# xkuubix/MonteCarlo-Gated-MIL

Measured on AMD Instinct MI355X. Metric: bags/sec × MCDO-samples (T=100) at N=2048,d=512; 1/2/4/8-GPU + %HBM roofline, higher is better.
Workload: dtype bf16

## Files before the change

montecarlo-gated-mil_amd/csrc/mcgmil_fused.hip:

```cpp
#define MCGMIL_KERNELS_TEMPLATES_ONLY
#include "../../include/mcgmil.h"
#include "mcgmil_kernels.h"
#include "mcgmil_error.h"
#include "mcgmil_fused.h"


namespace mcgmil {

__global__ __launch_bounds__(1024) void plan_regions_kernel(const int32_t* bag_off, int B, int T,
                                                            int cap, int32_t* region_off) {
    __shared__ int part[1024];
    const int tid = threadIdx.x;
    const int per = (B + 1023) / 1024;
    const int b0 = tid * per, b1 = b0 + per < B ? b0 + per : B;
    int sum = 0;
    for (int b = b0; b < b1; ++b) {
        const int ts = region_t_groups(bag_off[b + 1] - bag_off[b], T, cap);
        sum += (T + ts - 1) / ts;
    }
    part[tid] = sum;
    __syncthreads();
    for (int o = 1; o < 1024; o <<= 1) {
        const int v = tid >= o ? part[tid - o] : 0;
        __syncthreads();
        part[tid] += v;
        __syncthreads();
    }
    int run = part[tid] - sum;
    for (int b = b0; b < b1; ++b) {
        region_off[b] = run;
        const int ts = region_t_groups(bag_off[b + 1] - bag_off[b], T, cap);
        run += (T + ts - 1) / ts;
    }
    if (tid == 1023) region_off[B] = part[1023];
}

}

namespace mcgmil_detail {

long long fused_regions(const mcgmil::GateParams& gp, long long total_rows, int cap, bool estimate) {
    if (gp.uniform_rows > 0) {
        const int ts = mcgmil::region_t_groups(gp.uniform_rows, gp.T, cap);
        return (long long)gp.B * ((gp.T + ts - 1) / ts);
    }
    if (estimate) return (long long)gp.T * total_rows / cap;
    return (2ll * gp.T * total_rows + cap - 1) / cap + gp.B + 1;
}

namespace {

template <typename E, int PPW, int MAXC, bool ONE>
int launch(const mcgmil::GateParams& gp, long long total_rows, hipStream_t s) {
    constexpr int cap = mcgmil::fused_cap<MAXC>();
    const bool affine = mcgmil::fused_affine(gp.uniform_rows, cap);
    auto* k = affine ? (gp.clock ? &mcgmil::gate_fused_kernel<E, PPW, MAXC, ONE, true>
                                 : &mcgmil::gate_fused_kernel<E, PPW, MAXC, ONE>)
                     : (gp.clock ? &mcgmil::gate_fused_table_kernel<E, PPW, MAXC, ONE, true>
                                 : &mcgmil::gate_fused_table_kernel<E, PPW, MAXC, ONE>);
    if (int rc = raise_lds_limit(reinterpret_cast<const void*>(k), "gate_fused_kernel LDS limit")) return rc;
    if (gp.uniform_rows <= 0) {
        hipLaunchKernelGGL(mcgmil::plan_regions_kernel, dim3(1), dim3(1024), 0, s, gp.bag_off, gp.B,
                           gp.T, cap, const_cast<int32_t*>(gp.region_off));
        hipError_t e = hipGetLastError();
        if (e != hipSuccess) return hip_fail(e, "plan_regions_kernel launch");
    }
    const long long grid = fused_regions(gp, total_rows, cap, false);
    if (grid == 0) return MCGMIL_OK;
    if (grid > 0x7fffffffll) return fail(MCGMIL_E_UNSUPPORTED, "too many regions for one launch");
    const size_t lds = mcgmil::fused_kernel_lds_bytes<E, MAXC>(gp.L);
    if (lds > 160 * 1024) return fail(MCGMIL_E_UNSUPPORTED, "fused kernel: L too large for its LDS");
    hipLaunchKernelGGL(k, dim3((unsigned)grid), dim3(mcgmil::kGateThreads), lds, s, gp);
    hipError_t e = hipGetLastError();
    return e == hipSuccess ? MCGMIL_OK : hip_fail(e, "gate_fused_kernel launch");
}

template <typename E, int MAXC>
int launch_maxc(const mcgmil::GateParams& gp, int ppw, bool one, long long total_rows, hipStream_t s) {
    if (ppw == 1) return one ? launch<E, 1, MAXC, true>(gp, total_rows, s) : launch<E, 1, MAXC, false>(gp, total_rows, s);
    return one ? launch<E, 2, MAXC, true>(gp, total_rows, s) : launch<E, 2, MAXC, false>(gp, total_rows, s);
}

}

int launch_gate_fused(const mcgmil::GateParams& gp, bool bf16, int ppw, int maxc, bool one,
                      long long total_rows, hipStream_t s) {
    if (bf16) return maxc == 2 ? launch_maxc<__bf16, 2>(gp, ppw, one, total_rows, s)
                               : launch_maxc<__bf16, 4>(gp, ppw, one, total_rows, s);
    return maxc == 2 ? launch_maxc<float, 2>(gp, ppw, one, total_rows, s)
                     : launch_maxc<float, 4>(gp, ppw, one, total_rows, s);
}

}
```

montecarlo-gated-mil_amd/csrc/mcgmil_kernels.h:

```cpp
#pragma once
#include "mcgmil_device.h"

namespace mcgmil {

struct GateParams {
    const void* H;
    long long ldh;
    const int32_t* bag_off;
    int B, T, L, D, C, G, P;
    long long total_samples;
    const void* Wp;
    uint32_t wp_bytes;
    const float* bv;
    const float* bu;
    const float* wa;
    const float* ba;
    float sf, sa;
    uint32_t thr_f, thr_a;
    uint32_t thrx_f;
    uint32_t k0, k1;
    uint32_t bag_base;
    int t_base;
    const uint32_t* bag_ids;
    const int32_t* tile_bag;
    int uniform_rows;
    const uint8_t* keep_feat;
    const uint8_t* keep_att;
    float* logits;
    float* zz;
    float* Y;
    float* A;
    const int32_t* region_off;
    int region_t;
    unsigned long long* stamps;
    unsigned long long* clock;
    long long tile_row0;
};

constexpr int kClockSlots = 1024;
__device__ __forceinline__ void clock_probe(const GateParams& p, int i) {
    if (p.clock && threadIdx.x == 0 && blockIdx.x < (unsigned)kClockSlots) {
        const unsigned long long t = __builtin_amdgcn_s_memtime();
        const unsigned long long r = __builtin_amdgcn_s_memrealtime();
        p.clock[(size_t)blockIdx.x * 4 + 2 * i] = t;
        p.clock[(size_t)blockIdx.x * 4 + 2 * i + 1] = r;
    }
}

#ifdef MCGMIL_STAMPS
#define MCGMIL_STAMP(p, i)                                                                 \
    do {                                                                                    \
        __builtin_amdgcn_sched_barrier(0);                                                  \
        if (threadIdx.x == 0 && (p).stamps)                                                 \
            (p).stamps[(size_t)blockIdx.x * 8 + (i)] = __builtin_amdgcn_s_memtime();        \
        __builtin_amdgcn_sched_barrier(0);                                                  \
    } while (0)
#else
#define MCGMIL_STAMP(p, i) do {} while (0)
#endif


constexpr int kGateThreads = 512;
constexpr int kGateWaves = kGateThreads / kWave;
constexpr int kRowInfo = 6;


template <int BM, int RV = BM>
__device__ __forceinline__ void fill_row_table(const GateParams& p, long long R0, int* rinfo) {
    const int tid = threadIdx.x;
    if (tid >= BM) return;
    const long long R = tid < RV ? R0 + tid : p.total_samples;
    int hrow = -1, t = 0, n = 0, bag = 0, Nb = 0;
    const bool narrow = p.total_samples <= 0xFFFFFFFFll;
    if (R < p.total_samples && p.uniform_rows > 0) {
        const long long per_bag = (long long)p.T * p.uniform_rows;
        Nb = p.uniform_rows;
        if (narrow) {
            const uint32_t r = (uint32_t)R, pb = (uint32_t)per_bag;
            bag = (int)(r / pb);
            const uint32_t local = r - (uint32_t)bag * pb;
            t = (int)(local / (uint32_t)Nb);
            n = (int)(local - (uint32_t)t * (uint32_t)Nb);
        } else {
// ... 11 lines not shown
            bag = find_bag(p.bag_off, p.B, p.T, R);
        }
        const int ob = p.bag_off[bag];
        Nb = p.bag_off[bag + 1] - ob;
        const long long local = R - (long long)p.T * ob;
        if (narrow) {
            t = (int)((uint32_t)local / (uint32_t)Nb);
            n = (int)((uint32_t)local - (uint32_t)t * (uint32_t)Nb);
        } else {
            t = (int)(local / Nb);
            n = (int)(local - (long long)t * Nb);
        }
        hrow = ob + n;
    }
    int* ri = rinfo + kRowInfo * tid;
    ri[0] = hrow; ri[1] = t; ri[2] = n; ri[3] = bag; ri[4] = Nb;
    ri[5] = (int)(p.bag_ids ? p.bag_ids[bag] : p.bag_base + (uint32_t)bag);
}

#ifndef MCGMIL_KERNELS_TEMPLATES_ONLY
__global__ void plan_tiles_kernel(const int32_t* bag_off, int B, int T, long long total_samples,
                                  int BM, long long tiles, int32_t* tile_bag) {
    const long long i = (long long)blockIdx.x * blockDim.x + threadIdx.x;
    if (i >= tiles) return;
    const long long R = i * BM;
    tile_bag[i] = R < total_samples ? find_bag(bag_off, B, T, R) : 0;
}
#endif

__device__ __forceinline__ float gated_product_scaled(float ax, float by) {
    ax = fminf(fmaxf(ax, -43.280851226668903f), 43.280851226668903f);
    const float a = __builtin_amdgcn_exp2f(ax);
    const float b = __builtin_amdgcn_exp2f(by);
    const float ia = 1.0f + a;
    return (1.0f - a) * __builtin_amdgcn_rcpf(fmaf(ia, b, ia));
}

#ifndef MCGMIL_DIAG
#define MCGMIL_DIAG 0
#endif
#ifndef MCGMIL_PHILOX_ROUNDS
#define MCGMIL_PHILOX_ROUNDS 10
#endif

constexpr float kM2Log2e = -2.8853900817779268f;
constexpr float kMLog2e = -1.4426950408889634f;

struct HeadVec { f32x4 bv, bu, wa; };

template <int PPW>
__device__ __forceinline__ void load_head_vectors(const GateParams& p, int q0, int lane,
                                                  HeadVec (&hv)[PPW]) {
    const int DB = p.D >> 4;
#pragma unroll
    for (int jp = 0; jp < PPW; ++jp) {
        const int q = q0 + jp < p.P ? q0 + jp : p.P - 1;
        const int g = q / DB, db = q - g * DB;
        const int d0 = db * 16 + 4 * (lane >> 4);
        hv[jp].bv = *reinterpret_cast<const f32x4*>(p.bv + (size_t)g * p.D + d0) * kM2Log2e;
        hv[jp].bu = *reinterpret_cast<const f32x4*>(p.bu + (size_t)g * p.D + d0) * kMLog2e;
        hv[jp].wa = *reinterpret_cast<const f32x4*>(p.wa + (size_t)g * p.D + d0);
    }
}

struct Region {
    int bag, t0, t1, Nb, ob;
    int ntiles;
    long long S, rows;
};

constexpr int kFusedTiles = 32;
constexpr int kFusedHv = 256;
struct alignas(16) FusedConst {
    Region rg;
    uint32_t bagctr;
    int pad0;
    float ba[4];
    int cls[8];
    int pad1[8];
    int4 tile[kFusedTiles];
    float hv[3][kFusedHv];
};

#ifndef MCGMIL_FUSED_HV_LDS
#define MCGMIL_FUSED_HV_LDS 1
#endif
template <int PPW>
__device__ __forceinline__ void load_head_vectors_lds(const FusedConst* fc, int P, int q0, int lane,
                                                      HeadVec (&hv)[PPW]) {
#pragma unroll
    for (int jp = 0; jp < PPW; ++jp) {
        const int q = q0 + jp < P ? q0 + jp : P - 1;
        const int d = 16 * q + 4 * (lane >> 4);
        hv[jp].bv = *reinterpret_cast<const f32x4*>(fc->hv[0] + d);
        hv[jp].bu = *reinterpret_cast<const f32x4*>(fc->hv[1] + d);
        hv[jp].wa = *reinterpret_cast<const f32x4*>(fc->hv[2] + d);
    }
}

template <int RT, int PPW, int MAXC, bool ONE_CLASS, int RTV = RT>
__device__ __forceinline__ void fold_pairs(const GateParams& p, const f32x4 (&acc)[RT][2 * PPW],
                                           int q0, int lane, float (&part)[MAXC][RT],
                                           const HeadVec* pre = nullptr) {
    const int DB = p.D >> 4;
    const float av_s = p.sf * kM2Log2e, au_s = p.sf * kMLog2e;
#pragma unroll
    for (int jp = 0; jp < PPW; ++jp) {
        const int q = q0 + jp;
        if (q >= p.P) break;
        const int col = 16 * q + 4 * (lane >> 4);
        const int g = ONE_CLASS ? 0 : q / DB;
        const int d0 = col - g * p.D;
        f32x4 bvv, buv;
        f32x4 coef[MAXC];
        if (ONE_CLASS && pre) {
            bvv = pre[jp].bv;
            buv = pre[jp].bu;
            coef[0] = pre[jp].wa;
#pragma unroll
            for (int c = 1; c < MAXC; ++c) coef[c] = f32x4{0.f, 0.f, 0.f, 0.f};
        } else {
            bvv = *reinterpret_cast<const f32x4*>(p.bv + col);
            buv = *reinterpret_cast<const f32x4*>(p.bu + col);
            bvv *= kM2Log2e;
            buv *= kMLog2e;
#pragma unroll
            for (int c = 0; c < MAXC; ++c) {
                const int cc = ONE_CLASS ? g : c;
                const bool use = ONE_CLASS ? (c == 0) : ((c < p.C) && (p.G == 1 || c == g));
                const f32x4 w = *reinterpret_cast<const f32x4*>(p.wa + (size_t)(use ? cc : 0) * p.D + d0);
                coef[c] = use ? w : f32x4{0.f, 0.f, 0.f, 0.f};
            }
        }
#pragma unroll
        for (int rt = 0; rt < RTV; ++rt) {
#pragma unroll
            for (int v = 0; v < 4; ++v) {
                const float ax = fmaf(acc[rt][2 * jp][v], av_s, bvv[v]);
                const float by = fmaf(acc[rt][2 * jp + 1][v], au_s, buv[v]);
                if constexpr (ONE_CLASS) {
#if MCGMIL_DIAG & 8
                    part[0][rt] = fmaf(fmaf(ax, coef[0][v], by), ax, part[0][rt]);
                    continue;
#endif
                    const float a = __builtin_amdgcn_exp2f(fminf(fmaxf(ax, -43.280851226668903f),
                                                                 43.280851226668903f));
                    const float b = __builtin_amdgcn_exp2f(by);
                    const float ia = 1.0f + a;
                    const float r = __builtin_amdgcn_rcpf(fmaf(ia, b, ia));
                    part[0][rt] = fmaf(fmaf(-a, coef[0][v], coef[0][v]), r, part[0][rt]);
                } else {
                    const float pr = gated_product_scaled(ax, by);
#pragma unroll
                    for (int c = 0; c < MAXC; ++c) part[c][rt] = fmaf(pr, coef[c][v], part[c][rt]);
                }
            }
        }
    }
}

template <int BM, int MAXC>
__host__ __device__ constexpr int red_floats() { return kGateWaves * MAXC * 4 * BM; }

template <int BM, int MAXC, int ROWS = 16, bool AFFINE = false>
__device__ __forceinline__ void finish_scores(const GateParams& p, long long R0,
                                              float (&part)[MAXC][BM / ROWS], f32x4 zacc,
                                              bool zwave, float* red, float* zred,
                                              const int* rinfo, int one_class, int waves_per_gate,
                                              bool have_keep, bool keep, float* lg_out,
                                              float* z_out, long long obase,
                                              const FusedConst* fc = nullptr, int tile = 0) {
    constexpr int RT = BM / ROWS;
    constexpr int NG = 64 / ROWS;
    const int tid = threadIdx.x, lane = tid & 63, wave = tid >> 6;
    const int ncls = one_class < 0 ? MAXC : 1;
#pragma unroll
    for (int c = 0; c < MAXC; ++c) {
        if (c >= ncls) break;
        const int cls = one_class < 0 ? c : one_class;
        if (cls >= MAXC) break;
        float* dst = red + ((size_t)(wave * MAXC + cls) * NG + lane / ROWS) * BM + (lane % ROWS);
#pragma unroll
        for (int q = 0; q < RT; ++q) dst[ROWS * q] = part[c][q];
    }
    if (zwave && lane < 16) {
#pragma unroll
        for (int c = 0; c < MAXC; ++c) zred[c * BM + wave * 16 + lane] = zacc[c];
    }
    MCGMIL_STAMP(p, 5);
    __syncthreads();
    MCGMIL_STAMP(p, 6);
    const int r = wave * 16 + (lane & 15), c = lane >> 4;
    if (r >= BM || c >= p.C) return;
    int t, n, bag, Nb;
    uint32_t bagc;
    size_t orow;
    float bias;
    if constexpr (AFFINE) {
        const int4 tl = fc->tile[tile];
        t = tl.x, n = tl.y + r, bag = fc->rg.bag, Nb = fc->rg.Nb;
        bagc = fc->bagctr;
        orow = (size_t)(tl.z + r);
        bias = fc->ba[c];
    } else {
        const int* ri = rinfo + kRowInfo * r;
        if (ri[0] < 0) return;
        t = ri[1], n = ri[2], bag = ri[3], Nb = ri[4];
        bagc = (uint32_t)ri[5];
        orow = (size_t)(R0 + r - obase);
        bias = p.ba[c];
    }
    float s = 0.f;
    const int nw = waves_per_gate ? waves_per_gate : kGateWaves;
    for (int k = 0; k < nw; ++k) {
        const int w = waves_per_gate ? c * waves_per_gate + k : k;
        const float* src = red + (size_t)(w * MAXC + c) * NG * BM + r;
#pragma unroll
        for (int g = 0; g < NG; ++g) s += src[g * BM];
    }
    s += bias;
    if (p.keep_att) {
        const size_t abase = (size_t)p.T * p.C * (size_t)p.bag_off[bag];
        keep = p.keep_att[abase + ((size_t)t * p.C + c) * Nb + n] != 0;
    } else if (!have_keep) {
        keep = attention_keep(p.k0, p.k1, bagc, (uint32_t)(p.t_base + t), (uint32_t)c,
                              (uint32_t)n, p.thr_a);
    }
    const size_t o = orow * p.C + c;
    lg_out[o] = s * (keep ? p.sa : 0.f);
    z_out[o] = zred[c * BM + r] * p.sf;
}

constexpr int kSoftmaxRows = 16;

#ifndef MCGMIL_NT_A
#define MCGMIL_NT_A 1
#endif
__device__ __forceinline__ void store_a(float* dst, float v) {
#if MCGMIL_NT_A
    __builtin_nontemporal_store(v, dst);
#else
    *dst = v;
#endif
}

__device__ __forceinline__ void softmax_group(int ltid, bool active, int Nb, int C, const float* lg,
                                              const float* zz, float* Ao, float* Yo, float* sred) {
    const int tid = ltid, lane = ltid & 63, wave = ltid >> 6;
    if (Nb == 0) {
        if (active && tid < C) Yo[tid] = 0.f;
        return;
    }
    const int Nl = active ? Nb : 0;
    if (C == 2 && Nb <= 256 * kSoftmaxRows) {
        float (*sred2)[4] = reinterpret_cast<float (*)[4]>(sred);
        float e0[kSoftmaxRows], e1[kSoftmaxRows];
        float2 zr[kSoftmaxRows];
        float m0 = -INFINITY, m1 = -INFINITY;
#pragma unroll
        for (int k = 0; k < kSoftmaxRows; ++k) {
            const int n = tid + 256 * k;
            float2 l = make_float2(-INFINITY, -INFINITY);
            zr[k] = make_float2(0.f, 0.f);
            if (n < Nl) {
                l = *reinterpret_cast<const float2*>(lg + (size_t)n * 2);
                zr[k] = *reinterpret_cast<const float2*>(zz + (size_t)n * 2);
            }
            e0[k] = l.x;
            e1[k] = l.y;
            m0 = fmaxf(m0, e0[k]);
            m1 = fmaxf(m1, e1[k]);
        }
        m0 = wave_max(m0);
        m1 = wave_max(m1);
        if (lane == 0) { sred2[0][wave] = m0; sred2[1][wave] = m1; }
        __syncthreads();
        m0 = fmaxf(fmaxf(sred2[0][0], sred2[0][1]), fmaxf(sred2[0][2], sred2[0][3]));
        m1 = fmaxf(fmaxf(sred2[1][0], sred2[1][1]), fmaxf(sred2[1][2], sred2[1][3]));
        __syncthreads();
        float s0 = 0.f, y0 = 0.f, s1 = 0.f, y1 = 0.f;
#pragma unroll
        for (int k = 0; k < kSoftmaxRows; ++k) {
            const int n = tid + 256 * k;
            if (n < Nl) {
                const float2 z = zr[k];
                e0[k] = expf(e0[k] - m0);
                e1[k] = expf(e1[k] - m1);
                s0 += e0[k];
                s1 += e1[k];
                y0 = fmaf(e0[k], z.x, y0);
                y1 = fmaf(e1[k], z.y, y1);
            }
        }
        s0 = wave_sum(s0);
        y0 = wave_sum(y0);
        s1 = wave_sum(s1);
        y1 = wave_sum(y1);
        if (lane == 0) {
            sred2[0][wave] = s0; sred2[1][wave] = y0; sred2[2][wave] = s1; sred2[3][wave] = y1;
        }
        __syncthreads();
        s0 = (sred2[0][0] + sred2[0][1]) + (sred2[0][2] + sred2[0][3]);
        y0 = (sred2[1][0] + sred2[1][1]) + (sred2[1][2] + sred2[1][3]);
        s1 = (sred2[2][0] + sred2[2][1]) + (sred2[2][2] + sred2[2][3]);
        y1 = (sred2[3][0] + sred2[3][1]) + (sred2[3][2] + sred2[3][3]);
        __syncthreads();
// ... 106 lines not shown
template <> struct Raw<__bf16> { uint4 v; };
template <> struct Raw<float> { f32x4 lo, hi; };
__device__ __forceinline__ Raw<__bf16> load_raw(const __bf16* p) {
    Raw<__bf16> r; r.v = *reinterpret_cast<const uint4*>(p); return r;
}
__device__ __forceinline__ Raw<float> load_raw(const float* p) {
    Raw<float> r;
    r.lo = *reinterpret_cast<const f32x4*>(p);
    r.hi = *reinterpret_cast<const f32x4*>(p + 4);
    return r;
}
__device__ __forceinline__ void store_masked(const Raw<__bf16>& h, uint32_t kb, __bf16* dst) {
    uint4 v = h.v;
    v.x &= ((kb & 1u) ? 0x0000FFFFu : 0u) | ((kb & 2u) ? 0xFFFF0000u : 0u);
    v.y &= ((kb & 4u) ? 0x0000FFFFu : 0u) | ((kb & 8u) ? 0xFFFF0000u : 0u);
    v.z &= ((kb & 16u) ? 0x0000FFFFu : 0u) | ((kb & 32u) ? 0xFFFF0000u : 0u);
    v.w &= ((kb & 64u) ? 0x0000FFFFu : 0u) | ((kb & 128u) ? 0xFFFF0000u : 0u);
    *reinterpret_cast<uint4*>(dst) = v;
}
__device__ __forceinline__ void store_masked(const Raw<float>& h, uint32_t kb, float* dst) {
    f32x4 a = h.lo, b = h.hi;
    a.x = (kb & 1u) ? a.x : 0.f;   a.y = (kb & 2u) ? a.y : 0.f;
    a.z = (kb & 4u) ? a.z : 0.f;   a.w = (kb & 8u) ? a.w : 0.f;
    b.x = (kb & 16u) ? b.x : 0.f;  b.y = (kb & 32u) ? b.y : 0.f;
    b.z = (kb & 64u) ? b.z : 0.f;  b.w = (kb & 128u) ? b.w : 0.f;
    *reinterpret_cast<f32x4*>(dst) = a;
    *reinterpret_cast<f32x4*>(dst + 4) = b;
}

__device__ __forceinline__ void store_dropped(const Raw<__bf16>& h, uint4 o, uint32_t thrx,
                                              uint32_t inval, __bf16* dst) {
    uint4 v = h.v;
    v.x = __builtin_amdgcn_bitop3_b32(v.x, drop_mask16x2_flipped(o.x, thrx), inval, 0x10);
    v.y = __builtin_amdgcn_bitop3_b32(v.y, drop_mask16x2(o.y, thrx), inval, 0x10);
    v.z = __builtin_amdgcn_bitop3_b32(v.z, drop_mask16x2_flipped(o.z, thrx), inval, 0x10);
    v.w = __builtin_amdgcn_bitop3_b32(v.w, drop_mask16x2(o.w, thrx), inval, 0x10);
    *reinterpret_cast<uint4*>(dst) = v;
}
__device__ __forceinline__ uint32_t keep_lo(uint32_t m) { return ~(uint32_t)((int32_t)(m << 16) >> 16); }
__device__ __forceinline__ uint32_t keep_hi(uint32_t m) { return ~(uint32_t)((int32_t)m >> 16); }
__device__ __forceinline__ void store_dropped(const Raw<float>& h, uint4 o, uint32_t thrx,
                                              uint32_t inval, float* dst) {
    const uint32_t m0 = drop_mask16x2_flipped(o.x, thrx) | inval, m1 = drop_mask16x2(o.y, thrx) | inval;
    const uint32_t m2 = drop_mask16x2_flipped(o.z, thrx) | inval, m3 = drop_mask16x2(o.w, thrx) | inval;
    f32x4 a = h.lo, b = h.hi;
    a.x = __uint_as_float(__float_as_uint(a.x) & keep_lo(m0));
    a.y = __uint_as_float(__float_as_uint(a.y) & keep_hi(m0));
    a.z = __uint_as_float(__float_as_uint(a.z) & keep_lo(m1));
    a.w = __uint_as_float(__float_as_uint(a.w) & keep_hi(m1));
    b.x = __uint_as_float(__float_as_uint(b.x) & keep_lo(m2));
    b.y = __uint_as_float(__float_as_uint(b.y) & keep_hi(m2));
    b.z = __uint_as_float(__float_as_uint(b.z) & keep_lo(m3));
    b.w = __uint_as_float(__float_as_uint(b.w) & keep_hi(m3));
    *reinterpret_cast<f32x4*>(dst) = a;
    *reinterpret_cast<f32x4*>(dst + 4) = b;
}

constexpr int kPipeBM = 128;
#ifndef MCGMIL_VPM
#define MCGMIL_VPM 2
#endif
constexpr int VPM = MCGMIL_VPM;
#ifndef MCGMIL_SCHED
#define MCGMIL_SCHED 0
#endif
constexpr int HD = 2;
template <typename E>
__host__ __device__ constexpr int pipe_slots() { return 2; }

template <typename E, int MAXC>
__host__ __device__ constexpr size_t pipe_lds_bytes() {
    return (size_t)pipe_slots<E>() * kPipeBM * 32 * sizeof(E) + (size_t)red_floats<kPipeBM, MAXC>() * 4 +
           (size_t)MAXC * kPipeBM * 4 + (size_t)kRowInfo * kPipeBM * 4;
}

template <typename E>
__device__ __forceinline__ void load_classifier_lds(__amdgpu_buffer_rsrc_t wrs, uint32_t zsoff, int KS, E* zw) {
    for (int i = threadIdx.x; i < KS * 64; i += kGateThreads)
        *reinterpret_cast<f32x4*>(zw + (size_t)i * 8) = __builtin_bit_cast(
            f32x4, __builtin_amdgcn_raw_buffer_load_b128(wrs, (uint32_t)i * 8u * (uint32_t)sizeof(E), zsoff, 0));
}

template <typename E, int PPW, int MAXC, bool REPLAY, bool ONE_CLASS, bool EARLY_HV = true,
          bool ZL = false, bool ZLOAD = true, int RTV = kPipeBM / 16, bool AFFINE = false>
__device__ __forceinline__ void pipe_tile(const GateParams& p, long long R0, E* Xs, float* red,
                                          float* zred, const int* rinfo, float* lg_out,
                                          float* z_out, long long obase, E* zw = nullptr,
                                          const FusedConst* fc = nullptr, int tile = 0) {
    constexpr int BM = kPipeBM;
    constexpr int RT = BM / 16;
    constexpr int NJ = 2 * PPW;
    constexpr int SLOT = RT * 64 * 8;
    const int tid = threadIdx.x, lane = tid & 63, wave = tid >> 6;
    const int KS = p.L >> 5;

    int hrow;
    uint32_t cn, ct, cb;
    if constexpr (AFFINE) {
        static_assert(!REPLAY, "the affine rows have no replay masks");
        const int4 tl = fc->tile[tile];
        cn = (uint32_t)(tl.y + wave * 16 + (lane & 15));
        hrow = fc->rg.ob + (int)cn;
        ct = (uint32_t)(p.t_base + tl.x);
        cb = fc->bagctr;
    } else {
        const int* ri = rinfo + kRowInfo * (wave * 16 + (lane & 15));
        hrow = ri[0];
        cn = (uint32_t)ri[2], ct = (uint32_t)(p.t_base + ri[1]), cb = (uint32_t)ri[5];
    }
    const bool valid = AFFINE || hrow >= 0;
    const int kq = lane >> 4;
    const E* hsrc = reinterpret_cast<const E*>(p.H) + (size_t)(valid ? hrow : 0) * p.ldh + kq * 8;
    const uint8_t* kfe = REPLAY ? p.keep_feat + (size_t)(valid ? R0 + wave * 16 + (lane & 15) : 0) *
                                                    (p.L >> 3) + kq
                                : nullptr;

    const uint32_t inval = valid ? 0u : 0xFFFFFFFFu;
    auto stage = [&](int s, const Raw<E>& h, E* slot) {
        if constexpr (REPLAY) {
            const uint32_t kb = kfe[(size_t)(s < KS ? s : KS - 1) * 4];
            store_masked(h, kb & ~inval, slot + tid * 8);
        } else {
#if MCGMIL_DIAG & 4
            const uint4 o = make_uint4(cn * 0x9E3779B9u + (uint32_t)s, ct ^ cb, cn + ct, (uint32_t)s * 77u);
#else
            const uint4 o = philox4x32_10<true, MCGMIL_PHILOX_ROUNDS>((uint32_t)(s * 4 + kq), cn, ct, cb, p.k0, p.k1);
#endif
            store_dropped(h, o, p.thrx_f, inval, slot + tid * 8);
        }
    };

    const __amdgpu_buffer_rsrc_t wrs = make_rsrc(p.Wp, p.wp_bytes);
    const uint32_t tile_bytes = (uint32_t)KS * 512u * (uint32_t)sizeof(E);
    constexpr uint32_t kStepBytes = 512u * (uint32_t)sizeof(E);
    const int q0 = __builtin_amdgcn_readfirstlane(wave) * PPW;
    uint32_t wsoff[NJ];
#pragma unroll
    for (int j = 0; j < NJ; ++j) {
        int q = q0 + (j >> 1);
        q = q < p.P ? q : p.P - 1;
        wsoff[j] = (uint32_t)(2 * q + (j & 1)) * tile_bytes;
    }
    const uint32_t zsoff = (uint32_t)(2 * p.P) * tile_bytes;
    const uint32_t lane_b = (uint32_t)lane * 8u * (uint32_t)sizeof(E);
    auto wfrag = [&](uint32_t soff) { return load_frag_buf<E>(wrs, lane_b, soff); };

    f32x4 acc[RT][NJ];
#pragma unroll
    for (int rt = 0; rt < RT; ++rt)
#pragma unroll
        for (int j = 0; j < NJ; ++j) acc[rt][j] = f32x4{0.f, 0.f, 0.f, 0.f};
    f32x4 zacc = {0.f, 0.f, 0.f, 0.f};

    auto kstep = [&](int s, const E* cur, E* nxt, const Frag<E> (&w)[NJ], const Frag<E>& z,
                     Frag<E> (&wn)[NJ], Frag<E>& zn, const Raw<E>& h, Raw<E>& hn) {
        const int s1 = s + 1 < KS ? s + 1 : KS - 1;
        const int sh = s + HD < KS ? s + HD : KS - 1;
#if MCGMIL_DIAG & 2
#pragma unroll
        for (int j = 0; j < NJ; ++j) wn[j] = w[j];
        zn = z;
#else
#pragma unroll
        for (int j = 0; j < NJ; ++j) wn[j] = wfrag(wsoff[j] + (uint32_t)s1 * kStepBytes);
        if constexpr (!ZL) zn = wfrag(zsoff + (uint32_t)s1 * kStepBytes);
#endif
#if MCGMIL_DIAG & 1
        hn = h;
#else
        if (RTV == RT || wave < RTV) hn = load_raw(hsrc + (size_t)sh * 32);
#endif
#pragma unroll
        for (int rt = 0; rt < RTV; ++rt) {
            const Frag<E> x = load_frag(cur + (size_t)(rt * 64 + lane) * 8);
#pragma unroll
            for (int j = 0; j < NJ; ++j) acc[rt][j] = mma(w[j], x, acc[rt][j]);
        }
        const Frag<E> xz = load_frag(cur + (size_t)tid * 8);
        if constexpr (ZL) zacc = mma(load_frag(zw + (size_t)(s * 64 + lane) * 8), xz, zacc);
        else zacc = mma(z, xz, zacc);
        if (RTV == RT || wave < RTV) stage(s + 1, h, nxt);
        if constexpr (sizeof(E) == 2 && PPW == 2) {
#if MCGMIL_SCHED == 1
            __builtin_amdgcn_sched_group_barrier(0x020, NJ + 2, 0);
            __builtin_amdgcn_sched_group_barrier(0x100, 3, 0);
#pragma unroll
            for (int rt = 0; rt < RT; ++rt) {
#pragma unroll
                for (int j = 0; j < NJ; ++j) {
                    __builtin_amdgcn_sched_group_barrier(0x008, 1, 0);
                    __builtin_amdgcn_sched_group_barrier(0x002, VPM, 0);
                }
                if (rt + 2 < RT) __builtin_amdgcn_sched_group_barrier(0x100, 1, 0);
            }
            __builtin_amdgcn_sched_group_barrier(0x008, 1, 0);
            __builtin_amdgcn_sched_group_barrier(0x002, VPM, 0);
#else
#pragma unroll
            for (int i = 0; i < RTV * NJ + 1; ++i) {
                __builtin_amdgcn_sched_group_barrier(0x008, 1, 0);
                __builtin_amdgcn_sched_group_barrier(0x002, VPM, 0);
            }
#endif
        }
#if MCGMIL_DIAG & 128
        asm volatile("s_waitcnt lgkmcnt(0)" ::: "memory");
#else
        __syncthreads();
#endif
    };

    constexpr bool kEarlyHV = EARLY_HV && ONE_CLASS && sizeof(E) == 2;
    HeadVec hvec[PPW];
    {
        Frag<E> wA[NJ], wB[NJ], zA, zB;
        Raw<E> hA{}, hB{};
        if (RTV == RT || wave < RTV) {
            hA = load_raw(hsrc);
            hB = load_raw(hsrc + 32);
        }
#pragma unroll
        for (int j = 0; j < NJ; ++j) wA[j] = wfrag(wsoff[j]);
        if constexpr (ZL) {
            if constexpr (ZLOAD) load_classifier_lds<E>(wrs, zsoff, KS, zw);
        } else {
            zA = wfrag(zsoff);
        }
        if (RTV == RT || wave < RTV) stage(0, hA, Xs);
        __syncthreads();
        MCGMIL_STAMP(p, 2);

        if constexpr (kEarlyHV) load_head_vectors<PPW>(p, q0, lane, hvec);
        kstep(0, Xs, Xs + SLOT, wA, zA, wB, zB, hB, hA);
        kstep(1, Xs + SLOT, Xs, wB, zB, wA, zA, hA, hB);
#if MCGMIL_DIAG & 16
        if (KS > 1000)
#endif
        for (int s = 2; s < KS; s += 2) {
            kstep(s, Xs, Xs + SLOT, wA, zA, wB, zB, hB, hA);
            kstep(s + 1, Xs + SLOT, Xs, wB, zB, wA, zA, hA, hB);
        }
    }
    MCGMIL_STAMP(p, 3);

    float part[MAXC][RT];
#pragma unroll
    for (int c = 0; c < MAXC; ++c)
#pragma unroll
        for (int rt = 0; rt < RT; ++rt) part[c][rt] = 0.f;
    constexpr bool kLdsHV = MCGMIL_FUSED_HV_LDS && AFFINE && ONE_CLASS && !kEarlyHV;
    if constexpr (kLdsHV) load_head_vectors_lds<PPW>(fc, p.P, q0, lane, hvec);
    fold_pairs<RT, PPW, MAXC, ONE_CLASS, RTV>(p, acc, q0, lane, part, kEarlyHV || kLdsHV ? hvec : nullptr);
    MCGMIL_STAMP(p, 4);
    int one_class = -1;
    if constexpr (ONE_CLASS && AFFINE) one_class = __builtin_amdgcn_readfirstlane(fc->cls[wave]);
    else if constexpr (ONE_CLASS) one_class = q0 < p.P ? q0 / (p.D >> 4) : MAXC;
    finish_scores<BM, MAXC, 16, AFFINE>(p, R0, part, zacc, true, red, zred, rinfo, one_class,
                                        ONE_CLASS ? (p.D >> 4) / PPW : 0, false, true, lg_out, z_out,
                                        obase, fc, tile);
    MCGMIL_STAMP(p, 7);
}

#ifndef MCGMIL_XCD_TILES
#define MCGMIL_XCD_TILES 1
#endif
__device__ __forceinline__ long long xcd_tile(unsigned b, unsigned n, int bags) {
#if MCGMIL_XCD_TILES
    const unsigned x = b & 7u, q = n >> 3, r = n & 7u;
    const unsigned l = (x < r ? x * (q + 1) : r * (q + 1) + (x - r) * q) + (b >> 3);
    return (long long)(bags >= 8 ? l : b);
#else
    (void)n;
    (void)bags;
    return (long long)b;
#endif
}

template <typename E, int PPW, int MAXC, bool REPLAY, bool ONE_CLASS, bool PROBE = false, int RTV = kPipeBM / 16>
__global__ __launch_bounds__(kGateThreads) void gate_pipe_kernel(const GateParams p) {
    extern __shared__ __attribute__((aligned(16))) unsigned char smem[];
    constexpr int BM = kPipeBM;
    E* Xs = reinterpret_cast<E*>(smem);
    float* red = reinterpret_cast<float*>(smem + (size_t)pipe_slots<E>() * BM * 32 * sizeof(E));
    float* zred = red + red_floats<BM, MAXC>();
    int* rinfo = reinterpret_cast<int*>(zred + MAXC * BM);
    const long long R0 = RTV == BM / 16 ? xcd_tile(blockIdx.x, gridDim.x, p.B) * BM
                                        : p.tile_row0 + (long long)blockIdx.x * (16 * RTV);

    if constexpr (PROBE) clock_probe(p, 0);
    MCGMIL_STAMP(p, 0);
    fill_row_table<BM, 16 * RTV>(p, R0, rinfo);
    __syncthreads();
    MCGMIL_STAMP(p, 1);
    pipe_tile<E, PPW, MAXC, REPLAY, ONE_CLASS, true, false, true, RTV>(p, R0, Xs, red, zred, rinfo, p.logits,
                                                                       p.zz, 0);
    if constexpr (PROBE) clock_probe(p, 1);
}

#ifndef MCGMIL_FUSED_XCD
#define MCGMIL_FUSED_XCD 1
#endif
#ifndef MCGMIL_FUSED_EARLY_HV
#define MCGMIL_FUSED_EARLY_HV 0
#endif
#ifndef MCGMIL_FUSED_NMAJOR
#define MCGMIL_FUSED_NMAJOR 1
#endif
#ifndef MCGMIL_FUSED_CAP
#define MCGMIL_FUSED_CAP 4096
#endif
template <int MAXC>
__host__ __device__ constexpr int fused_cap() { return MAXC <= 2 ? MCGMIL_FUSED_CAP : MCGMIL_FUSED_CAP / 4; }

template <typename E, int MAXC>
__host__ __device__ constexpr size_t fused_lds_bytes() {
    return pipe_lds_bytes<E, MAXC>() + (size_t)kRowInfo * kPipeBM * 4
           + (size_t)2 * fused_cap<MAXC>() * MAXC * 4
           + (size_t)2 * 16 * 4 + sizeof(FusedConst);
}
static_assert(kFusedTiles * kPipeBM >= MCGMIL_FUSED_CAP, "FusedConst::tile holds a whole region");

__host__ __device__ inline bool fused_affine(int uniform_rows, int cap) {
    return uniform_rows > 0 && uniform_rows % kPipeBM == 0 && uniform_rows <= cap;
}

#ifndef MCGMIL_FUSED_ZL
#define MCGMIL_FUSED_ZL 1
#endif
template <typename E>
__host__ __device__ constexpr bool fused_zl() { return MCGMIL_FUSED_ZL && sizeof(E) == 2; }
template <typename E, int MAXC>
__host__ __device__ constexpr size_t fused_kernel_lds_bytes(int L) {
    return fused_lds_bytes<E, MAXC>() + (fused_zl<E>() ? (size_t)(L / 32) * 512 * sizeof(E) : 0);
}

__host__ __device__ inline int region_t_groups(int Nb, int T, int cap) {
    if (Nb <= 0) return T;
    if (Nb > cap) return 1;
    const int ts = cap / Nb;
    return ts < T ? ts : T;
}

__device__ __forceinline__ int region_tile(const Region& rg, int i) {
#if MCGMIL_FUSED_NMAJOR
    const int G = rg.t1 - rg.t0;
    if (G > 1 && rg.Nb % kPipeBM == 0) return (i % G) * (rg.Nb / kPipeBM) + i / G;
#endif
    return i;
}

__device__ __forceinline__ GateParams reload_kernarg_params(const GateParams& p) {
#if __HIP_DEVICE_COMPILE__
    typedef __attribute__((address_space(4))) const GateParams* KernargParams;
    KernargParams q = (KernargParams)__builtin_amdgcn_kernarg_segment_ptr();
    asm volatile("" : "+s"(q));
    return *q;
#else
    return p;
#endif
}

__device__ __forceinline__ bool decode_region(const GateParams& p, int g, int cap, Region& rg) {
    int b, j, ts;
    if (p.uniform_rows > 0) {
        ts = p.region_t;
        const int rpb = (p.T + ts - 1) / ts;
        if (MCGMIL_FUSED_XCD && (p.B & 7) == 0) {
            const int k = g >> 3;
            b = 8 * (k / rpb) + (g & 7);
            j = k - (k / rpb) * rpb;
        } else {
            b = g / rpb;
            j = g - b * rpb;
        }
        if (b >= p.B) return false;
    } else {
        if (g >= p.region_off[p.B]) return false;
        b = find_bag(p.region_off, p.B, 1, g);
        j = g - p.region_off[b];
        ts = region_t_groups(p.bag_off[b + 1] - p.bag_off[b], p.T, cap);
    }
    rg.bag = b;
    rg.ob = p.bag_off[b];
    rg.Nb = p.bag_off[b + 1] - rg.ob;
    rg.t0 = j * ts;
    rg.t1 = rg.t0 + ts < p.T ? rg.t0 + ts : p.T;
    rg.S = (long long)p.T * rg.ob + (long long)rg.t0 * rg.Nb;
    rg.rows = (long long)(rg.t1 - rg.t0) * rg.Nb;
    rg.ntiles = (int)((rg.rows + kPipeBM - 1) / kPipeBM);
    return true;
}

template <int BM>
__device__ __forceinline__ void fill_row_table_region(const GateParams& p, const Region& rg,
                                                      long long R0, int* rinfo) {
    const int tid = threadIdx.x;
    if (tid >= BM) return;
    const long long rho = R0 + tid - rg.S;
    int hrow = -1, t = 0, n = 0;
    if (rho < rg.rows) {
        const uint32_t r = (uint32_t)rho;
        const uint32_t tt = r / (uint32_t)rg.Nb;
        n = (int)(r - tt * (uint32_t)rg.Nb);
        t = rg.t0 + (int)tt;
        hrow = rg.ob + n;
    }
    int* ri = rinfo + kRowInfo * tid;
    ri[0] = hrow; ri[1] = t; ri[2] = n; ri[3] = rg.bag; ri[4] = rg.Nb;
    ri[5] = (int)(p.bag_ids ? p.bag_ids[rg.bag] : p.bag_base + (uint32_t)rg.bag);
}


template <int PPW, int MAXC, bool ONE_CLASS>
__device__ __forceinline__ void fill_fused_const(const GateParams& p, const Region& rg, FusedConst* fc) {
    const int tid = threadIdx.x;
    if (tid == 0) {
        fc->rg = rg;
        fc->bagctr = p.bag_ids ? p.bag_ids[rg.bag] : p.bag_base + (uint32_t)rg.bag;
    }
    if (tid < MAXC) fc->ba[tid] = tid < p.C ? p.ba[tid] : 0.f;
    if (tid < kGateWaves) {
        const int q0 = tid * PPW, DB = p.D >> 4;
        int g = 0;
        while ((g + 1) * DB <= q0) ++g;
        fc->cls[tid] = ONE_CLASS && q0 < p.P ? g : MAXC;
    }
    if (tid < rg.ntiles && tid < kFusedTiles) {
        const int G = rg.t1 - rg.t0, nbt = rg.Nb / kPipeBM;
        const int dv = MCGMIL_FUSED_NMAJOR ? G : nbt;
        int qt = 0;
        while ((qt + 1) * dv <= tid) ++qt;
        const int rem = tid - qt * dv;
        const int tg = MCGMIL_FUSED_NMAJOR ? rem : qt, nb = MCGMIL_FUSED_NMAJOR ? qt : rem;
        fc->tile[tid] = make_int4(rg.t0 + tg, nb * kPipeBM, tg * rg.Nb + nb * kPipeBM, 0);
    }
    if (ONE_CLASS && tid < 16 * p.P && tid < kFusedHv) {
        fc->hv[0][tid] = p.bv[tid] * kM2Log2e;
        fc->hv[1][tid] = p.bu[tid] * kMLog2e;
        fc->hv[2][tid] = p.wa[tid];
    }
}

template <typename E, int PPW, int MAXC, bool ONE_CLASS, bool PROBE, bool AFFINE>
__device__ __forceinline__ void fused_region(const GateParams& p) {
    extern __shared__ __attribute__((aligned(16))) unsigned char smem[];
    constexpr int BM = kPipeBM;
    constexpr int CAP = fused_cap<MAXC>();
    E* Xs = reinterpret_cast<E*>(smem);
    float* red = reinterpret_cast<float*>(smem + (size_t)pipe_slots<E>() * BM * 32 * sizeof(E));
    float* zred = red + red_floats<BM, MAXC>();
    int* rinfo = reinterpret_cast<int*>(zred + MAXC * BM);
    float* slg = reinterpret_cast<float*>(rinfo + 2 * kRowInfo * BM);
    float* szz = slg + CAP * MAXC;
    float* sred = szz + CAP * MAXC;
    FusedConst* fc = reinterpret_cast<FusedConst*>(sred + 32);

#if MCGMIL_DIAG & 64
    {
        const long long R0 = (long long)blockIdx.x * BM;
        fill_row_table<BM>(p, R0, rinfo);
        __syncthreads();
        pipe_tile<E, PPW, MAXC, false, ONE_CLASS>(p, R0, Xs, red, zred, rinfo, p.logits, p.zz, 0);
        return;
    }
#endif
    Region rg;
    if (!decode_region(p, (int)blockIdx.x, CAP, rg)) return;
    if constexpr (PROBE) clock_probe(p, 0);
    const int ntiles = (int)((rg.rows + BM - 1) / BM);
    Region* srg = &fc->rg;
    if constexpr (AFFINE) fill_fused_const<PPW, MAXC, ONE_CLASS>(p, rg, fc);
    else if (threadIdx.x == 0) *srg = rg;
    __syncthreads();
    E* zw = reinterpret_cast<E*>(smem + fused_lds_bytes<E, MAXC>());
    if constexpr (fused_zl<E>())
        load_classifier_lds<E>(make_rsrc(p.Wp, p.wp_bytes), (uint32_t)(2 * p.P) * (uint32_t)(p.L >> 5) * 512u *
                                   (uint32_t)sizeof(E), p.L >> 5, zw);
    for (int i = 0; i < ntiles; ++i) {
        const GateParams pt = reload_kernarg_params(p);
        if constexpr (AFFINE) {
            MCGMIL_STAMP(pt, 0);
            MCGMIL_STAMP(pt, 1);
            pipe_tile<E, PPW, MAXC, false, ONE_CLASS, MCGMIL_FUSED_EARLY_HV, fused_zl<E>(), false, BM / 16, true>(
                pt, 0, Xs, red, zred, nullptr, slg, szz, 0, zw, fc, i);
        } else {
            Region* qr = srg;
            asm volatile("" : "+v"(qr));
            int* ri = rinfo + (i & 1) * kRowInfo * BM;
            MCGMIL_STAMP(pt, 0);
            {
                const Region r = *qr;
                fill_row_table_region<BM>(pt, r, r.S + (long long)region_tile(r, i) * BM, ri);
            }
            __syncthreads();
            MCGMIL_STAMP(pt, 1);
            const Region r = *qr;
            const bool lds = r.Nb <= CAP;
            pipe_tile<E, PPW, MAXC, false, ONE_CLASS, MCGMIL_FUSED_EARLY_HV, fused_zl<E>(), false>(
                pt, r.S + (long long)region_tile(r, i) * BM, Xs, red, zred, ri, lds ? slg : pt.logits,
                lds ? szz : pt.zz, lds ? r.S : 0, zw);
        }
    }
    __syncthreads();
#if MCGMIL_DIAG & 32
    if (ntiles >= 0) return;
#endif
    rg = *srg;
    const bool in_lds = AFFINE || rg.Nb <= CAP;

    const int G = rg.t1 - rg.t0;
    const int half = threadIdx.x >> 8, ltid = threadIdx.x & 255;
    for (int j0 = 0; j0 < G; j0 += 2) {
        const bool act = j0 + half < G;
        const int j = act ? j0 + half : j0;
        const long long row0 = (long long)j * rg.Nb;
        const float* lgj = in_lds ? slg + row0 * p.C : p.logits + (rg.S + row0) * p.C;
        const float* zzj = in_lds ? szz + row0 * p.C : p.zz + (rg.S + row0) * p.C;
        float* Ao = p.A ? p.A + (size_t)p.T * p.C * rg.ob + (size_t)(rg.t0 + j) * p.C * rg.Nb : nullptr;
        float* Yo = p.Y + ((size_t)rg.bag * p.T + rg.t0 + j) * p.C;
        softmax_group(ltid, act, rg.Nb, p.C, lgj, zzj, Ao, Yo, sred + half * 16);
    }
    if constexpr (PROBE) clock_probe(p, 1);
}

template <typename E, int PPW, int MAXC, bool ONE_CLASS, bool PROBE = false>
__global__ __launch_bounds__(kGateThreads) void gate_fused_kernel(const GateParams p) {
    fused_region<E, PPW, MAXC, ONE_CLASS, PROBE, true>(p);
}

template <typename E, int PPW, int MAXC, bool ONE_CLASS, bool PROBE = false>
__global__ __launch_bounds__(kGateThreads) void gate_fused_table_kernel(const GateParams p) {
    fused_region<E, PPW, MAXC, ONE_CLASS, PROBE, false>(p);
}

template <int BM>
__host__ __device__ constexpr int gate_row_info_ints() { return kRowInfo * BM; }

template <typename E, int BM, int MAXC>
__host__ __device__ constexpr size_t gate_lds_bytes(int L) {
    const size_t tile = (size_t)BM * L * sizeof(E), red = (size_t)red_floats<BM, MAXC>() * 4;
    return (tile > red ? tile : red) + (size_t)MAXC * BM * 4 + (size_t)gate_row_info_ints<BM>() * 4;
}

template <typename E, int BM, int PPW, int MAXC>
__global__ __launch_bounds__(kGateThreads) void gate_scores_kernel(const GateParams p) {
    extern __shared__ __attribute__((aligned(16))) unsigned char smem[];
    constexpr int RT = BM / 16;
    constexpr int NJ = 2 * PPW;
    const int tid = threadIdx.x;
    const int lane = tid & 63;
    const int wave = tid >> 6;
    const int L = p.L;
    const int KS = L >> 5;
    const int LC = L >> 3;

    E* Xs = reinterpret_cast<E*>(smem);
    float* red = reinterpret_cast<float*>(smem);
    const size_t tile_bytes = (size_t)BM * L * sizeof(E), red_bytes = (size_t)red_floats<BM, MAXC>() * 4;
    float* zred = reinterpret_cast<float*>(smem + (tile_bytes > red_bytes ? tile_bytes : red_bytes));
    int* rinfo = reinterpret_cast<int*>(zred + MAXC * BM);
    const long long R0 = (long long)blockIdx.x * BM;

    fill_row_table<BM>(p, R0, rinfo);
    __syncthreads();

    {
        const E* H = reinterpret_cast<const E*>(p.H);
        const int items = BM * LC;
        for (int i = tid; i < items; i += kGateThreads) {
            const int blk = i >> 6, slot = i & 63;
            const int rt = blk / KS, ks = blk - rt * KS;
            const int r = rt * 16 + (slot & 15);
            const int kc = ks * 4 + (slot >> 4);
            E* dst = Xs + ((size_t)blk * 64 + slot) * 8;
            const int* ri = rinfo + kRowInfo * r;
            const int hrow = ri[0];
            if (hrow < 0) {
                store_zero8(dst);
                continue;
            }
            uint32_t kb;
            if (p.keep_feat) {
                kb = p.keep_feat[(size_t)(R0 + r) * LC + kc];
            } else {
                const uint4 o = philox4x32_10((uint32_t)kc, (uint32_t)ri[2],
                                              (uint32_t)(p.t_base + ri[1]), (uint32_t)ri[5],
                                              p.k0, p.k1);
                kb = keep_byte(o, p.thr_f);
            }
            load_masked(H + (size_t)hrow * p.ldh + (size_t)kc * 8, kb, dst);
        }
    }
    __syncthreads();

    const E* Wp = reinterpret_cast<const E*>(p.Wp);
    const int pairs_per_pass = kGateWaves * PPW;
    const int npass = (p.P + pairs_per_pass - 1) / pairs_per_pass;
    const size_t tile_elems = (size_t)KS * 512;

    float part[MAXC][RT];
#pragma unroll
    for (int c = 0; c < MAXC; ++c)
#pragma unroll
        for (int rt = 0; rt < RT; ++rt) part[c][rt] = 0.f;
    f32x4 zacc = {0.f, 0.f, 0.f, 0.f};
    const bool zwave = wave < RT;

    for (int pass = 0; pass < npass; ++pass) {
        const int q0 = pass * pairs_per_pass + wave * PPW;
        const bool active = q0 < p.P;
// ... 201 lines not shown
```

Baseline: 976,800.

## Precompute dropout keep masks in LDS and add async H-image prefetch kernel

Before the tile loop, each block now computes the attention-dropout keep bits once per tile and class with philox and stores them in LDS, overlaid on the row tables. finish_scores then reads these bits instead of regenerating random numbers per element. It also adds an optional kernel variant that uses buffer-load-to-LDS DMA to prefetch the next tile's H rows into an LDS image while the current tile computes. That variant is disabled by default (MCGMIL_FUSED_H_IMAGE=0), so only the keep-mask precompute is active on the default path, at the cost of extra LDS and a one-time upfront philox pass.

```diff
diff --git a/montecarlo-gated-mil_amd/csrc/mcgmil_fused.hip b/montecarlo-gated-mil_amd/csrc/mcgmil_fused.hip
--- a/montecarlo-gated-mil_amd/csrc/mcgmil_fused.hip
+++ b/montecarlo-gated-mil_amd/csrc/mcgmil_fused.hip
@@ -58,6 +58,13 @@
                                  : &mcgmil::gate_fused_kernel<E, PPW, MAXC, ONE>)
                      : (gp.clock ? &mcgmil::gate_fused_table_kernel<E, PPW, MAXC, ONE, true>
                                  : &mcgmil::gate_fused_table_kernel<E, PPW, MAXC, ONE>);
+    size_t lds = mcgmil::fused_kernel_lds_bytes<E, MAXC>(gp.L);
+    if constexpr (mcgmil::fused_image_type<E>()) {
+        if (affine && !gp.clock && mcgmil::fused_image_ok<E, MAXC>(gp.L, gp.uniform_rows, gp.ldh)) {
+            k = &mcgmil::gate_fused_image_kernel<E, PPW, MAXC, ONE>;
+            lds += mcgmil::kFusedImageBytes;
+        }
+    }
     if (int rc = raise_lds_limit(reinterpret_cast<const void*>(k), "gate_fused_kernel LDS limit")) return rc;
     if (gp.uniform_rows <= 0) {
         hipLaunchKernelGGL(mcgmil::plan_regions_kernel, dim3(1), dim3(1024), 0, s, gp.bag_off, gp.B,
@@ -68,8 +75,7 @@
     const long long grid = fused_regions(gp, total_rows, cap, false);
     if (grid == 0) return MCGMIL_OK;
     if (grid > 0x7fffffffll) return fail(MCGMIL_E_UNSUPPORTED, "too many regions for one launch");
-    const size_t lds = mcgmil::fused_kernel_lds_bytes<E, MAXC>(gp.L);
-    if (lds > 160 * 1024) return fail(MCGMIL_E_UNSUPPORTED, "fused kernel: L too large for its LDS");
+    if (lds > mcgmil::kFusedLdsLimit) return fail(MCGMIL_E_UNSUPPORTED, "fused kernel: L too large for its LDS");
     hipLaunchKernelGGL(k, dim3((unsigned)grid), dim3(mcgmil::kGateThreads), lds, s, gp);
     hipError_t e = hipGetLastError();
     return e == hipSuccess ? MCGMIL_OK : hip_fail(e, "gate_fused_kernel launch");
diff --git a/montecarlo-gated-mil_amd/csrc/mcgmil_kernels.h b/montecarlo-gated-mil_amd/csrc/mcgmil_kernels.h
--- a/montecarlo-gated-mil_amd/csrc/mcgmil_kernels.h
+++ b/montecarlo-gated-mil_amd/csrc/mcgmil_kernels.h
@@ -1,4 +1,5 @@
 #pragma once
+#include <type_traits>
 #include "mcgmil_device.h"
 
 namespace mcgmil {
@@ -176,6 +177,52 @@
     float hv[3][kFusedHv];
 };
 
+#ifndef MCGMIL_FUSED_KEEP_LDS
+#define MCGMIL_FUSED_KEEP_LDS 1
+#endif
+constexpr int kFusedKeepBytes = 4 * kFusedTiles * 16;
+static_assert(kFusedKeepBytes <= 2 * kRowInfo * 128 * 4, "the keep bytes overlay the two row tables");
+__device__ __forceinline__ int keep_slot(int tile, int c, int octet) {
+    return (c * kFusedTiles + tile) * 16 + octet;
+}
+
+#ifndef MCGMIL_FUSED_H_IMAGE
+#define MCGMIL_FUSED_H_IMAGE 0
+#endif
+constexpr size_t kFusedImageBytes = (size_t)2 * 512 * 16;
+
+__device__ __forceinline__ void dma16_lds(__amdgpu_buffer_rsrc_t r, void* lds, uint32_t voff, uint32_t soff) {
+#if defined(__HIP_DEVICE_COMPILE__)
+    __builtin_amdgcn_raw_ptr_buffer_load_lds(r, (__attribute__((address_space(3))) void*)lds, 16, voff, soff, 0, 0);
+#else
+    (void)r; (void)lds; (void)voff; (void)soff;
+#endif
+}
+
+static_assert(kFusedKeepBytes + kFusedTiles * 16 <= 2 * kRowInfo * 128 * 4, "keep bytes + image records overlay the row tables");
+__device__ __forceinline__ uint4* image_records(uint8_t* keepa) {
+    return reinterpret_cast<uint4*>(keepa + kFusedKeepBytes);
+}
+__device__ __forceinline__ const uint4* image_records(const uint8_t* keepa) {
+    return reinterpret_cast<const uint4*>(keepa + kFusedKeepBytes);
+}
+
+template <typename E>
+__device__ __forceinline__ void issue_h_image(const GateParams& p, const uint4* rec, int tile, E* img) {
+    static_assert(sizeof(E) == 2, "the image holds 16-byte chunks (bf16)");
+    const int tid = threadIdx.x, lane = tid & 63;
+    const int wave = __builtin_amdgcn_readfirstlane(tid >> 6);
+    const uint4 r = rec[tile];
+    const uint32_t row0 = __builtin_amdgcn_readfirstlane(r.x), range = __builtin_amdgcn_readfirstlane(r.w);
+    const uint64_t base = (uint64_t)(uint32_t)__builtin_amdgcn_readfirstlane(r.y) |
+                          (uint64_t)(uint32_t)__builtin_amdgcn_readfirstlane(r.z) << 32;
+    const uint32_t row_b = (uint32_t)p.ldh * (uint32_t)sizeof(E);
+    const __amdgpu_buffer_rsrc_t rs = make_rsrc(reinterpret_cast<const void*>(base), range);
+    const uint32_t voff = (uint32_t)(wave * 16 + (lane & 15)) * row_b + (uint32_t)(lane >> 4) * 16u;
+    dma16_lds(rs, img + (size_t)wave * 512, voff, row0);
+    dma16_lds(rs, img + (size_t)(4096 + wave * 512), voff, row0 + 64u);
+}
+
 #ifndef MCGMIL_FUSED_HV_LDS
 #define MCGMIL_FUSED_HV_LDS 1
 #endif
@@ -263,7 +310,8 @@
                                               const int* rinfo, int one_class, int waves_per_gate,
                                               bool have_keep, bool keep, float* lg_out,
                                               float* z_out, long long obase,
-                                              const FusedConst* fc = nullptr, int tile = 0) {
+                                              const FusedConst* fc = nullptr, int tile = 0,
+                                              const uint8_t* keepa = nullptr) {
     constexpr int RT = BM / ROWS;
     constexpr int NG = 64 / ROWS;
     const int tid = threadIdx.x, lane = tid & 63, wave = tid >> 6;
@@ -316,6 +364,8 @@
     if (p.keep_att) {
         const size_t abase = (size_t)p.T * p.C * (size_t)p.bag_off[bag];
         keep = p.keep_att[abase + ((size_t)t * p.C + c) * Nb + n] != 0;
+    } else if (AFFINE && MCGMIL_FUSED_KEEP_LDS) {
+        keep = (keepa[keep_slot(tile, c, r >> 3)] >> (n & 7)) & 1;
     } else if (!have_keep) {
         keep = attention_keep(p.k0, p.k1, bagc, (uint32_t)(p.t_base + t), (uint32_t)c,
                               (uint32_t)n, p.thr_a);
@@ -588,11 +638,13 @@
 }
 
 template <typename E, int PPW, int MAXC, bool REPLAY, bool ONE_CLASS, bool EARLY_HV = true,
-          bool ZL = false, bool ZLOAD = true, int RTV = kPipeBM / 16, bool AFFINE = false>
+          bool ZL = false, bool ZLOAD = true, int RTV = kPipeBM / 16, bool AFFINE = false, bool IMG = false>
 __device__ __forceinline__ void pipe_tile(const GateParams& p, long long R0, E* Xs, float* red,
                                           float* zred, const int* rinfo, float* lg_out,
                                           float* z_out, long long obase, E* zw = nullptr,
-                                          const FusedConst* fc = nullptr, int tile = 0) {
+                                          const FusedConst* fc = nullptr, int tile = 0,
+                                          const uint8_t* keepa = nullptr, E* img = nullptr, bool more = false) {
+    static_assert(!IMG || (AFFINE && RTV == kPipeBM / 16), "the H image belongs to the affine launch");
     constexpr int BM = kPipeBM;
     constexpr int RT = BM / 16;
     constexpr int NJ = 2 * PPW;
@@ -721,7 +773,10 @@
     {
         Frag<E> wA[NJ], wB[NJ], zA, zB;
         Raw<E> hA{}, hB{};
-        if (RTV == RT || wave < RTV) {
+        if constexpr (IMG) {
+            hA = load_raw(img + (size_t)tid * 8);
+            hB = load_raw(img + (size_t)(SLOT + tid * 8));
+        } else if (RTV == RT || wave < RTV) {
             hA = load_raw(hsrc);
             hB = load_raw(hsrc + 32);
         }
@@ -756,14 +811,17 @@
         for (int rt = 0; rt < RT; ++rt) part[c][rt] = 0.f;
     constexpr bool kLdsHV = MCGMIL_FUSED_HV_LDS && AFFINE && ONE_CLASS && !kEarlyHV;
     if constexpr (kLdsHV) load_head_vectors_lds<PPW>(fc, p.P, q0, lane, hvec);
-    fold_pairs<RT, PPW, MAXC, ONE_CLASS, RTV>(p, acc, q0, lane, part, kEarlyHV || kLdsHV ? hvec : nullptr);
-    MCGMIL_STAMP(p, 4);
     int one_class = -1;
     if constexpr (ONE_CLASS && AFFINE) one_class = __builtin_amdgcn_readfirstlane(fc->cls[wave]);
     else if constexpr (ONE_CLASS) one_class = q0 < p.P ? q0 / (p.D >> 4) : MAXC;
+    if constexpr (IMG) {
+        if (more) issue_h_image<E>(p, image_records(keepa), tile + 1, img);
+    }
+    fold_pairs<RT, PPW, MAXC, ONE_CLASS, RTV>(p, acc, q0, lane, part, kEarlyHV || kLdsHV ? hvec : nullptr);
+    MCGMIL_STAMP(p, 4);
     finish_scores<BM, MAXC, 16, AFFINE>(p, R0, part, zacc, true, red, zred, rinfo, one_class,
                                         ONE_CLASS ? (p.D >> 4) / PPW : 0, false, true, lg_out, z_out,
-                                        obase, fc, tile);
+                                        obase, fc, tile, keepa);
     MCGMIL_STAMP(p, 7);
 }
 
@@ -839,6 +897,30 @@
 __host__ __device__ constexpr size_t fused_kernel_lds_bytes(int L) {
     return fused_lds_bytes<E, MAXC>() + (fused_zl<E>() ? (size_t)(L / 32) * 512 * sizeof(E) : 0);
 }
+
+constexpr size_t kFusedLdsLimit = 160 * 1024;
+template <typename E>
+__host__ __device__ constexpr bool fused_image_type() { return MCGMIL_FUSED_H_IMAGE && sizeof(E) == 2; }
+template <typename E, int MAXC>
+__host__ __device__ constexpr bool fused_image_ok(int L, int uniform_rows, long long ldh) {
+    return fused_image_type<E>() && fused_kernel_lds_bytes<E, MAXC>(L) + kFusedImageBytes <= kFusedLdsLimit &&
+           (long long)uniform_rows * ldh * (long long)sizeof(E) <= 0xFFFFFFFFll;
+}
+template <typename E, int MAXC>
+__host__ __device__ constexpr size_t fused_affine_lds_bytes(int L) {
+    return fused_kernel_lds_bytes<E, MAXC>(L) + (fused_image_ok<E, MAXC>(L, kPipeBM, L) ? kFusedImageBytes : 0);
+}
+template <typename E, int MAXC>
+__host__ __device__ constexpr bool fused_lds_fits() {
+    for (int L = 128; L <= 8192; L += 64)
+        if (fused_kernel_lds_bytes<E, MAXC>(L) <= kFusedLdsLimit && fused_affine_lds_bytes<E, MAXC>(L) > kFusedLdsLimit)
+            return false;
+    return true;
+}
+static_assert(fused_lds_fits<__bf16, 2>() && fused_lds_fits<__bf16, 4>() && fused_lds_fits<float, 2>() &&
+                  fused_lds_fits<float, 4>(), "a fused launch the host admits exceeds the CU's LDS");
+static_assert(!MCGMIL_FUSED_H_IMAGE || (fused_image_ok<__bf16, 2>(512, 2048, 512) && !fused_image_ok<__bf16, 2>(1024, 256, 1024)),
+              "H image: on at L = 512, off from L = 1024");
 
 __host__ __device__ inline int region_t_groups(int Nb, int T, int cap) {
     if (Nb <= 0) return T;
@@ -917,8 +999,9 @@
 }
 
 
-template <int PPW, int MAXC, bool ONE_CLASS>
-__device__ __forceinline__ void fill_fused_const(const GateParams& p, const Region& rg, FusedConst* fc) {
+template <int PPW, int MAXC, bool ONE_CLASS, typename E = void>
+__device__ __forceinline__ void fill_fused_const(const GateParams& p, const Region& rg, FusedConst* fc,
+                                                 uint4* rec = nullptr) {
     const int tid = threadIdx.x;
     if (tid == 0) {
         fc->rg = rg;
@@ -939,6 +1022,12 @@
         const int rem = tid - qt * dv;
         const int tg = MCGMIL_FUSED_NMAJOR ? rem : qt, nb = MCGMIL_FUSED_NMAJOR ? qt : rem;
         fc->tile[tid] = make_int4(rg.t0 + tg, nb * kPipeBM, tg * rg.Nb + nb * kPipeBM, 0);
+        if constexpr (!std::is_void<E>::value) {
+            const uint32_t row_b = (uint32_t)p.ldh * (uint32_t)sizeof(E);
+            const uint64_t base = (uint64_t)reinterpret_cast<uintptr_t>(p.H) + (uint64_t)rg.ob * p.ldh * sizeof(E);
+            rec[tid] = make_uint4((uint32_t)(nb * kPipeBM) * row_b, (uint32_t)base, (uint32_t)(base >> 32),
+                                  (uint32_t)(rg.Nb - 1) * row_b + (uint32_t)p.L * (uint32_t)sizeof(E));
+        }
     }
     if (ONE_CLASS && tid < 16 * p.P && tid < kFusedHv) {
         fc->hv[0][tid] = p.bv[tid] * kM2Log2e;
@@ -947,11 +1036,25 @@
     }
 }
 
-template <typename E, int PPW, int MAXC, bool ONE_CLASS, bool PROBE, bool AFFINE>
+__device__ __forceinline__ void fill_fused_keeps(const GateParams& p, const FusedConst* fc, uint8_t* keepa) {
+    const int tile = threadIdx.x >> 4, octet = threadIdx.x & 15;
+    static_assert(kGateThreads == kFusedTiles * 16, "one thread per (tile, octet)");
+    if (tile >= fc->rg.ntiles) return;
+    const int4 tl = fc->tile[tile];
+    for (int c = 0; c < p.C; ++c) {
+        const uint4 o = philox4x32_10((uint32_t)((tl.y >> 3) + octet), (uint32_t)c,
+                                      (uint32_t)(p.t_base + tl.x) | 0x80000000u, fc->bagctr, p.k0, p.k1);
+        keepa[keep_slot(tile, c, octet)] = (uint8_t)keep_byte(o, p.thr_a);
+    }
+}
+
+template <typename E, int PPW, int MAXC, bool ONE_CLASS, bool PROBE, bool AFFINE, bool IMG = false>
 __device__ __forceinline__ void fused_region(const GateParams& p) {
-    extern __shared__ __attribute__((aligned(16))) unsigned char smem[];
+    extern __shared__ __attribute__((aligned(16))) unsigned char lds[];
     constexpr int BM = kPipeBM;
     constexpr int CAP = fused_cap<MAXC>();
+    E* img = reinterpret_cast<E*>(lds);
+    unsigned char* smem = lds + (IMG ? kFusedImageBytes : 0);
     E* Xs = reinterpret_cast<E*>(smem);
     float* red = reinterpret_cast<float*>(smem + (size_t)pipe_slots<E>() * BM * 32 * sizeof(E));
     float* zred = red + red_floats<BM, MAXC>();
@@ -975,20 +1078,29 @@
     if constexpr (PROBE) clock_probe(p, 0);
     const int ntiles = (int)((rg.rows + BM - 1) / BM);
     Region* srg = &fc->rg;
-    if constexpr (AFFINE) fill_fused_const<PPW, MAXC, ONE_CLASS>(p, rg, fc);
+    uint8_t* keepa = reinterpret_cast<uint8_t*>(rinfo);
+    if constexpr (IMG) fill_fused_const<PPW, MAXC, ONE_CLASS, E>(p, rg, fc, image_records(keepa));
+    else if constexpr (AFFINE) fill_fused_const<PPW, MAXC, ONE_CLASS>(p, rg, fc);
     else if (threadIdx.x == 0) *srg = rg;
     __syncthreads();
     E* zw = reinterpret_cast<E*>(smem + fused_lds_bytes<E, MAXC>());
+    if constexpr (IMG) issue_h_image<E>(p, image_records(keepa), 0, img);
+    if constexpr (AFFINE && MCGMIL_FUSED_KEEP_LDS) fill_fused_keeps(p, fc, keepa);
     if constexpr (fused_zl<E>())
         load_classifier_lds<E>(make_rsrc(p.Wp, p.wp_bytes), (uint32_t)(2 * p.P) * (uint32_t)(p.L >> 5) * 512u *
                                    (uint32_t)sizeof(E), p.L >> 5, zw);
     for (int i = 0; i < ntiles; ++i) {
+#if defined(MCGMIL_STAMPS) && defined(MCGMIL_STAMPS_INNER)
+        GateParams pt = reload_kernarg_params(p);
+        if (ntiles > 1 && i + 1 == ntiles) pt.stamps = nullptr;
+#else
         const GateParams pt = reload_kernarg_params(p);
+#endif
         if constexpr (AFFINE) {
             MCGMIL_STAMP(pt, 0);
             MCGMIL_STAMP(pt, 1);
-            pipe_tile<E, PPW, MAXC, false, ONE_CLASS, MCGMIL_FUSED_EARLY_HV, fused_zl<E>(), false, BM / 16, true>(
-                pt, 0, Xs, red, zred, nullptr, slg, szz, 0, zw, fc, i);
+            pipe_tile<E, PPW, MAXC, false, ONE_CLASS, MCGMIL_FUSED_EARLY_HV, fused_zl<E>(), false, BM / 16, true, IMG>(
+                pt, 0, Xs, red, zred, nullptr, slg, szz, 0, zw, fc, i, keepa, img, i + 1 < ntiles);
         } else {
             Region* qr = srg;
             asm volatile("" : "+v"(qr));
@@ -1032,6 +1144,11 @@
 template <typename E, int PPW, int MAXC, bool ONE_CLASS, bool PROBE = false>
 __global__ __launch_bounds__(kGateThreads) void gate_fused_kernel(const GateParams p) {
     fused_region<E, PPW, MAXC, ONE_CLASS, PROBE, true>(p);
+}
+
+template <typename E, int PPW, int MAXC, bool ONE_CLASS>
+__global__ __launch_bounds__(kGateThreads) void gate_fused_image_kernel(const GateParams p) {
+    fused_region<E, PPW, MAXC, ONE_CLASS, false, true, true>(p);
 }
 
 template <typename E, int PPW, int MAXC, bool ONE_CLASS, bool PROBE = false>
```

New measurement: 982,400 (median of 6 runs). No clear change (+0.6%).
